# CX9898/BSMR-SDDMM

Measured on AMD Instinct MI355X. Metric: SDDMM GFLOP/s, higher is better.
Workload: dtype f16

## Files before the change

### bsmr-sddmm_amd/csrc/bsmr_capi.hip

```cpp

#include "bsmr_hip.h"

#include <hip/hip_runtime.h>
#include <hipcub/hipcub.hpp>

#include <algorithm>
#include <chrono>
#include <cmath>
#include <cstdio>
#include <cstdlib>
#include <cstring>
#include <map>
#include <memory>
#include <mutex>
#include <new>
#include <set>
#include <string>
#include <vector>

#include "cluster_kernels.hpp"
#include "pack_device.hpp"
#include "promote_device.hpp"
#include "plan_pack.hpp"
#include "plan_promote.hpp"
// ... 35 lines not shown
    uint32_t* groupRows = nullptr;
    uint32_t* blockCols = nullptr;
    uint32_t* blockInfo = nullptr;
    uint32_t* entries = nullptr;
    bsmr::TileItem* items = nullptr;
    uint32_t* itemRowBase = nullptr;
    uint32_t numItems = 0, entryCap = 0, blocksPerItem = 0;
    uint64_t numBlocks = 0, numTiles = 0, unionColumns = 0, bytes = 0;
};

struct SweepFormatDev {
    uint32_t W = 0, PW = 0, stripBlocks = 0;
    uint32_t* panelRows = nullptr;
    bsmr::SweepItem* items = nullptr;
    uint32_t* starts = nullptr;
    uint32_t* rowStart = nullptr;
    uint32_t* words = nullptr;
    uint32_t numItems = 0, numGroups = 0, numStrips = 0, maxStepEntries = 0, maxItemWords = 0;
    uint64_t bytes = 0;
    bool usable = false;
};

struct GemmFormatDev {
    uint32_t PM = 0, NB = 0;
    uint32_t* panelRows = nullptr;
    uint32_t* colOf = nullptr;
    bsmr::GemmItem* items = nullptr;
    uint32_t* rowStart = nullptr;
    uint32_t* lists = nullptr;
    uint32_t* words = nullptr;
    uint32_t numItems = 0, numGroups = 0, numStrips = 0;
    uint64_t numTiles = 0, bytes = 0;
    bool fullGrid = false, usable = false;
};

struct bsmr_plan {
    int device = 0;
    uint32_t M = 0, N = 0, nnz = 0, numPanels = 0;

    DenseFormat fmt[2];
    uint64_t numDenseEntries = 0;

    uint32_t* panelRows = nullptr;
    uint32_t* entryCol = nullptr;
    uint32_t* entryDst = nullptr;
    uint8_t* entryRow = nullptr;
    SparseItem* sparseItems = nullptr;
    uint64_t numSparseEntries = 0;
    uint32_t numSparseItems = 0;

    uint64_t indexBytes = 0;

    uint16_t* A16 = nullptr;
    uint16_t* B16 = nullptr;
    uint32_t reservedK = 0;

    int sparseLpe = 0;
    bool sparseLowp = true;
    bool convertInKernel = false;
    uint32_t* entryRowId = nullptr;
    bool sparseFree = false;
    uint64_t foldedEntries = 0;
    uint64_t promotedEntries = 0;
    uint64_t evictedEntries = 0;
    bool groupedDeferred = false;
    bsmr::PackOptions groupedOpt;
    float buildMs[5] = {0, 0, 0, 0, 0};
    bool packedOnDevice = false;
    bool promotedOnDevice = false;
    bool convertPass = false;
    bool convertBOnly = false;
    uint64_t bOnlyWork = 0;
    int denseBatch = 0;
    bool useStream = true;

    bsmr::HostDense hostDense;
    mutable bsmr::TileCensus census[5];
    mutable bool censusDone[5] = {false, false, false, false, false};
    TileFormatDev tiles[5];
    bool useTiles = false;
    bool sharedB = false;
    bool tunable = false;
    std::vector<SweepFormatDev> sweeps;
    bool useSweep = false;
    int sweepNow = -1;
    int sweepPanelsNow = 0, sweepBlocksNow = 0, sweepWavesNow = 0, sweepPerCuNow = 0;
    std::vector<GemmFormatDev> gemms;
    bool useGemm = false;
    int gemmNow = -1;
    int gemmPanelsNow = 0, gemmBlocksNow = 0;
    struct Tuned {
        int engine = BSMR_ENGINE_STREAM, group = 0, blocksPerItem = 0;
        int format = -1;
        int bOnly = -1;
        int overlap = -1;
        int cvt = -1;
        int waves = 0;
    };
    std::map<uint64_t, Tuned> tuned;
    int tileGroupNow = 0, tileBlocksNow = 0;
    int formatNow = -1, bOnlyNow = -1, overlapNow = -1, cvtNow = -1;
    bsmr_plan_options opt{};

    bool overlap = false;
    hipStream_t sideStream = nullptr;
    hipEvent_t forkEvent = nullptr, joinEvent = nullptr;

    struct Retained {
        bsmr_rphm_desc desc{};
        std::vector<uint32_t> reorderedRows, denseCols, blockOffsets, blockValues, sparseOffsets, sparseValues, sparseRows, sparseCols;
    };
    std::unique_ptr<Retained> retained;
    bsmr_plan* delegate = nullptr;
    uint64_t delegateKey = 0;
    int variantChosen = 0;
};

namespace {

constexpr uint64_t kGroupedGatherBytes = 400ull << 20;

thread_local std::string g_lastHipError;
inline bsmr_plan* served(bsmr_plan* p) { return p && p->delegate ? p->delegate : p; }
// ... 1071 lines not shown
    if (src32) {
        switch (K) {
        case 32: return launchSweepP<1, MODE, true>(w, p->device, perCu, p->N, A, B, P, s);
        case 64: return launchSweepP<2, MODE, true>(w, p->device, perCu, p->N, A, B, P, s);
        case 128: return launchSweepP<4, MODE, true>(w, p->device, perCu, p->N, A, B, P, s);
        default: return BSMR_ERR_INVALID_ARG;
        }
    }
    switch (K) {
    case 32: return launchSweepP<1, MODE, false>(w, p->device, perCu, p->N, A, B, P, s);
    case 64: return launchSweepP<2, MODE, false>(w, p->device, perCu, p->N, A, B, P, s);
    case 128: return launchSweepP<4, MODE, false>(w, p->device, perCu, p->N, A, B, P, s);
    case 256: return launchSweepP<8, MODE, false>(w, p->device, perCu, p->N, A, B, P, s);
    case 512: return launchSweepP<16, MODE, false>(w, p->device, perCu, p->N, A, B, P, s);
    default: return BSMR_ERR_INVALID_ARG;
    }
}

inline bool gemmServesK(uint32_t K) { return K == 64 || K == 128 || K == 256 || K == 512; }
inline bool gemmFp32ServesK(uint32_t K) { return K == 64 || K == 128; }
inline bool gemmFits(const bsmr_plan* p, uint32_t K, uint32_t elemBytes = 2) {
    return (uint64_t)p->M * K * elemBytes < (1ull << 32) && (uint64_t)p->N * K * elemBytes < (1ull << 32) &&
           (uint64_t)p->nnz * 4u <= 0xFFFFFFFCull;
}
inline bool gemmWanted(const bsmr_plan* p, uint32_t K) {
    return p->useGemm && gemmServesK(K) && gemmFits(p, K) && p->hostDense.entries() != 0;
}
inline bool gemmEngine(const bsmr_plan* p) { return p->gemmNow >= 0; }
inline bool gemmFp32(const bsmr_plan* p, uint32_t K) {
    if (!gemmFp32ServesK(K) || !gemmFits(p, K, 4)) return false;
    if (p->cvtNow >= 0) return p->cvtNow == 1;
    return p->opt.gemm_fp32 > 0 || (p->opt.gemm_fp32 < 0 && p->numSparseItems == 0);
}
constexpr uint32_t kGemmShapes[][2] = {{16, 16}, {16, 20}, {16, 12}, {8, 16}, {8, 20}};
inline double gemmModelUs(const bsmr_plan* p, uint32_t K, uint32_t PM, uint32_t NB) {
    const uint64_t G = (p->numPanels + PM - 1) / PM, S = ((p->N + 15u) / 16u + NB - 1) / NB;
    const double perCu = PM * NB <= 160 ? 2.0 : 1.0;
    const double rounds = std::ceil((double)(G * S) / (256.0 * perCu));
    const double slice = 1.4 * (PM * NB / 256.0) * (PM * NB < 256 ? 1.15 : 1.0) * perCu;
    return 2.0 + rounds * (4.0 + slice * (K / 64.0));
}
inline bool gemmShapeBuilt(uint32_t PM, uint32_t NB, bool fp32 = false) {
    for (const auto& sh : kGemmShapes)
        if (sh[0] == PM && sh[1] == NB) return !(fp32 && NB == 12);
    return false;
}
void gemmShape(const bsmr_plan* p, uint32_t K, uint32_t& PM, uint32_t& NB, int rank = 0) {
    const int forcedPM = p->gemmPanelsNow > 0 ? p->gemmPanelsNow : p->opt.gemm_panels;
    const int forcedNB = p->gemmBlocksNow > 0 ? p->gemmBlocksNow : p->opt.gemm_blocks;
    if (forcedPM > 0 && forcedNB > 0) {
        PM = (uint32_t)forcedPM;
        NB = (uint32_t)forcedNB;
        return;
    }
    std::vector<std::pair<double, uint32_t>> order;
    const bool fp32 = gemmFp32(p, K);
    for (uint32_t i = 0; i < sizeof(kGemmShapes) / sizeof(kGemmShapes[0]); ++i)
        if (gemmShapeBuilt(kGemmShapes[i][0], kGemmShapes[i][1], fp32))
            order.push_back({gemmModelUs(p, K, kGemmShapes[i][0], kGemmShapes[i][1]), i});
    std::stable_sort(order.begin(), order.end());
    const uint32_t pick = order[std::min<size_t>((size_t)rank, order.size() - 1)].second;
    PM = kGemmShapes[pick][0];
    NB = kGemmShapes[pick][1];
}

int ensureGemm(bsmr_plan* p, uint32_t K) {
    uint32_t PM, NB;
    gemmShape(p, K, PM, NB);
    p->gemmNow = -1;
    if (!gemmShapeBuilt(PM, NB, gemmFp32(p, K))) return BSMR_OK;
    for (size_t i = 0; i < p->gemms.size(); ++i)
        if (p->gemms[i].PM == PM && p->gemms[i].NB == NB) {
            if (p->gemms[i].usable) p->gemmNow = (int)i;
            return BSMR_OK;
        }
    try {
        GemmFormatDev w;
        w.PM = PM;
        w.NB = NB;
        bsmr::GemmFormatHost host;
        int st = bsmr::packGemm(p->hostDense, PM, NB, host, p->opt.gemm_balance_columns != 0);
        if (st == BSMR_ERR_BAD_PLAN || st == BSMR_ERR_INVALID_ARG) {
            p->gemms.push_back(w);
            return BSMR_OK;
        }
        if (st != BSMR_OK) return st;
        uint64_t bytes = 0;
        w.numItems = (uint32_t)host.items.size();
        w.numGroups = host.numGroups;
        w.numStrips = host.numStrips;
        w.numTiles = host.numTiles;
        w.fullGrid = host.fullGrid;
        st = upload(w.panelRows, host.panelRows, bytes);
        if (st == BSMR_OK) st = upload(w.colOf, host.colOf, bytes);
        if (st == BSMR_OK) st = upload(w.items, host.items, bytes);
        if (st == BSMR_OK) st = upload(w.rowStart, host.rowStart, bytes);
        if (st == BSMR_OK) st = upload(w.lists, host.lists, bytes);
        if (st == BSMR_OK) st = upload(w.words, host.words, bytes);
        if (st != BSMR_OK) {
            void* wp[] = {w.panelRows, w.colOf, w.items, w.rowStart, w.lists, w.words};
            for (void* q : wp)
                if (q) (void)hipFree(q);
            return st;
        }
        w.bytes = bytes;
        w.usable = w.numItems != 0;
        p->indexBytes += bytes;
        p->gemms.push_back(w);
        if (w.usable) p->gemmNow = (int)p->gemms.size() - 1;
        return BSMR_OK;
    } catch (const std::bad_alloc&) {
        return BSMR_ERR_OOM;
    }
}

template <int KT, int PM, int NB, int MODE, bool SRC32>
int launchGemmT(const GemmFormatDev& w, const bsmr_plan* p, const void* A, const void* B, float* P, const Queue& s) {
    const uint64_t K = (SRC32 ? 32u : 64u) * KT, esz = SRC32 ? 4 : 2;
    const uint32_t aBytes = (uint32_t)((uint64_t)p->M * K * esz), bBytes = (uint32_t)((uint64_t)p->N * K * esz);
    const dim3 grid(w.numItems, s.batch.count), block(bsmr::kGemmWaves * bsmr::kWave);
    if constexpr (SRC32) {
        auto kernel = bsmr::denseGemmCvt<KT, PM, NB, MODE>;
        const size_t lds = bsmr::gemmCvtLdsBytes(PM, NB);
        if (int st = raiseDynamicLds(reinterpret_cast<const void*>(kernel), lds, p->device)) return st;
        hipLaunchKernelGGL(kernel, grid, block, lds, s, static_cast<const float*>(A), static_cast<const float*>(B), aBytes, bBytes, w.panelRows,
                           w.colOf, w.items, w.rowStart, w.lists, w.words, P, p->N, w.numGroups, w.numStrips, w.fullGrid ? 1u : 0u, s.batch);
    } else {
        auto kernel = bsmr::denseGemm<KT, PM, NB, MODE, false>;
        const size_t lds = bsmr::gemmLdsBytes(PM, NB);
        if (int st = raiseDynamicLds(reinterpret_cast<const void*>(kernel), lds, p->device)) return st;
        hipLaunchKernelGGL(kernel, grid, block, lds, s, A, B, aBytes, bBytes, w.panelRows, w.colOf, w.items, w.rowStart, w.lists, w.words, P, p->N,
                           w.numGroups, w.numStrips, w.fullGrid ? 1u : 0u, s.batch);
    }
    BSMR_HIP(hipGetLastError());
    return BSMR_OK;
}
template <int KT, int MODE, bool SRC32>
int launchGemmS(const GemmFormatDev& w, const bsmr_plan* p, const void* A, const void* B, float* P, const Queue& s) {
    switch (w.PM * 100 + w.NB) {
    case 1616: return launchGemmT<KT, 16, 16, MODE, SRC32>(w, p, A, B, P, s);
    case 1620: return launchGemmT<KT, 16, 20, MODE, SRC32>(w, p, A, B, P, s);
    case 816: return launchGemmT<KT, 8, 16, MODE, SRC32>(w, p, A, B, P, s);
    case 820: return launchGemmT<KT, 8, 20, MODE, SRC32>(w, p, A, B, P, s);
    case 1612:
        if constexpr (!SRC32) return launchGemmT<KT, 16, 12, MODE, false>(w, p, A, B, P, s);
        return BSMR_ERR_INVALID_ARG;
    default: return BSMR_ERR_INVALID_ARG;
    }
}
template <int MODE>
int launchGemm(const bsmr_plan* p, uint32_t K, const void* A, const void* B, float* P, const Queue& s, bool src32) {
    const GemmFormatDev& w = p->gemms[(size_t)p->gemmNow];
    if (w.numItems == 0) return BSMR_OK;
    if (src32) {
        switch (K) {
        case 64: return launchGemmS<2, MODE, true>(w, p, A, B, P, s);
        case 128: return launchGemmS<4, MODE, true>(w, p, A, B, P, s);
        default: return BSMR_ERR_INVALID_ARG;
        }
    }
    switch (K) {
    case 64: return launchGemmS<1, MODE, false>(w, p, A, B, P, s);
    case 128: return launchGemmS<2, MODE, false>(w, p, A, B, P, s);
    case 256: return launchGemmS<4, MODE, false>(w, p, A, B, P, s);
    case 512: return launchGemmS<8, MODE, false>(w, p, A, B, P, s);
    default: return BSMR_ERR_INVALID_ARG;
    }
}

inline bool streamCvtServes(const DenseFormat& f, uint32_t K) {
    return (K == 32 || K == 64 || K == 128) && f.H == 1 && f.maxItemBlocks <= 8 && (f.tiles8 || f.tilesM) && !f.stageInLds;
// ... 221 lines not shown
        return BSMR_ERR_INVALID_ARG;
    return BSMR_OK;
}

bool aligned16(const void* p) { return ((uintptr_t)p & 15u) == 0; }
bool aligned4(const void* p) { return ((uintptr_t)p & 3u) == 0; }

int checkDeviceCall(const bsmr_plan* p, uint32_t K, const void* A, const void* B, const void* P, int mode) {
    if (int st = checkCall(p, K, A, B, P, mode)) return st;
    return aligned16(A) && aligned16(B) && aligned4(P) ? BSMR_OK : BSMR_ERR_INVALID_ARG;
}

inline bool convertsBOnly(const bsmr_plan* p, uint32_t K, uint32_t batches = 1) {
    if (!p->convertBOnly || (size_t)16 * (2u * K + bsmr::kSparseLdsPad16) > 64 * 1024) return false;
    if (p->bOnlyNow >= 0) return p->bOnlyNow == 1;
    const uint64_t work = (uint64_t)p->numSparseEntries * K * batches;
    return work >= p->bOnlyWork || (p->numSparseEntries >= 11ull * p->N && work * 10 >= p->bOnlyWork * 3);
}

inline bool needsWorkspace(const bsmr_plan* p, int mode, uint32_t K, uint32_t batches = 1) {
    return mode != BSMR_COMPUTE_F32 && (convertPassOf(p, K) || convertsBOnly(p, K, batches));
}

int prepareDense(bsmr_plan* p, uint32_t K, int mode) {
    p->sweepNow = -1;
    p->gemmNow = -1;
    if (p->tunable) {
        const auto it = mode == BSMR_COMPUTE_F32 ? p->tuned.end() : p->tuned.find(((uint64_t)K << 8) | (uint32_t)mode);
        const bsmr_plan::Tuned choice = it == p->tuned.end() ? bsmr_plan::Tuned{} : it->second;
        p->useSweep = choice.engine == BSMR_ENGINE_SWEEP;
        p->useGemm = choice.engine == BSMR_ENGINE_GEMM;
        p->gemmPanelsNow = p->useGemm ? choice.group : 0;
        p->gemmBlocksNow = p->useGemm ? choice.blocksPerItem : 0;
        p->useTiles = choice.engine == BSMR_ENGINE_TILES || choice.engine == BSMR_ENGINE_SHARED;
        p->sharedB = choice.engine == BSMR_ENGINE_SHARED;
        p->tileGroupNow = p->useTiles ? choice.group : 0;
        p->tileBlocksNow = p->useTiles ? choice.blocksPerItem : 0;
        p->sweepPanelsNow = p->useSweep ? choice.group : 0;
        p->sweepBlocksNow = p->useSweep ? choice.blocksPerItem : 0;
        p->sweepWavesNow = p->useSweep ? choice.waves : 0;
        p->formatNow = choice.format;
        p->bOnlyNow = choice.bOnly;
        p->overlapNow = choice.overlap;
        p->cvtNow = choice.cvt;
    }
    if (mode == BSMR_COMPUTE_F32) return BSMR_OK;
    if (gemmWanted(p, K)) {
        if (int st = ensureGemm(p, K)) return st;
        if (gemmEngine(p)) return BSMR_OK;
    }
    if (sweepWanted(p, K)) {
        if (int st = ensureSweep(p, K)) return st;
        if (sweepEngine(p)) return BSMR_OK;
    }
    if (!tilesEngine(p, K)) return BSMR_OK;
    return ensureTiles(p, chooseTileGroup(p, K));
}

int reserve(bsmr_plan* p, uint32_t K) {
    if (p->reservedK >= K && p->A16 && p->B16) return BSMR_OK;
    if (p->A16) (void)hipFree(p->A16);
    if (p->B16) (void)hipFree(p->B16);
    p->A16 = p->B16 = nullptr;
    p->reservedK = 0;
    const size_t a = std::max<size_t>((size_t)p->M * K * 2, 16), b = std::max<size_t>((size_t)p->N * K * 2, 16);
    if (!hipOk(hipMalloc(reinterpret_cast<void**>(&p->A16), a), "hipMalloc(A16)")) return BSMR_ERR_OOM;
// ... 1124 lines not shown
        }
        if (st == BSMR_OK && r.lowp_call_us >= 0.f && r.sweep_fp32_call_us >= 0.f && r.sweep_fp32_call_us < r.lowp_call_us * kTuneMargin) {
            best = bestF;
            r.chosen_sweep_fp32 = 1;
        }
    }
    if (st == BSMR_OK && lowp && gemmFp32ServesK(K) && gemmFits(plan, K, 4) && plan->fmt[0].numItems && !plan->convertInKernel && sweepApplies(plan)) {
        float callUs = r.lowp_call_us;
        if (r.chosen_sweep_fp32 && r.sweep_fp32_call_us >= 0.f) callUs = r.sweep_fp32_call_us;
        if (callUs < 0.f) st = timeChoice(best, 7, callUs);
        bsmr_plan::Tuned f = best, bestF = best;
        f.engine = BSMR_ENGINE_GEMM;
        f.format = -1;
        f.cvt = 1;
        f.waves = 0;
        uint32_t seenPM = 0, seenNB = 0;
        for (int rank = 0; rank < 2 && st == BSMR_OK; ++rank) {
            uint32_t PM, NB;
            plan->gemmPanelsNow = plan->gemmBlocksNow = 0;
            plan->cvtNow = 1;
            gemmShape(plan, K, PM, NB, rank);
            if (PM == seenPM && NB == seenNB) continue;
            seenPM = PM;
            seenNB = NB;
            f.group = (int)PM;
            f.blocksPerItem = (int)NB;
            float us = -1.f;
            st = timeChoice(f, 7, us);
            if (st == BSMR_OK && us >= 0.f && (r.gemm_fp32_call_us < 0.f || us < r.gemm_fp32_call_us)) {
                r.gemm_fp32_call_us = us;
                bestF = f;
            }
        }
        if (st == BSMR_OK && callUs >= 0.f && r.gemm_fp32_call_us >= 0.f && r.gemm_fp32_call_us < callUs * kTuneMargin) {
            best = bestF;
            r.chosen_sweep_fp32 = 0;
            r.chosen_gemm_fp32 = 1;
        }
        if (r.lowp_call_us < 0.f) r.lowp_call_us = callUs;
    }
    if (st != BSMR_OK) {
        plan->tuned.erase(key);
        return st;
    }
    plan->tuned[key] = best;
    r.chosen_cvt_in_kernel = best.cvt;
    r.chosen_engine = best.engine;
    r.chosen_group = best.engine == BSMR_ENGINE_STREAM ? (best.format == 1 ? (int)plan->fmt[1].H : 1) : best.group;
    r.chosen_blocks_per_item = best.blocksPerItem;
    r.chosen_b_only = best.bOnly;
    r.chosen_overlap = best.overlap;
    if ((st = prepareDense(plan, K, mode)) != BSMR_OK) return st;
    if (best.engine == BSMR_ENGINE_SWEEP && sweepEngine(plan)) r.chosen_blocks_per_item = (int)plan->sweeps[(size_t)plan->sweepNow].stripBlocks;
    if (needsWorkspace(plan, mode, K) && (st = reserve(plan, K)) != BSMR_OK) return st;
    st = runPieces(plan, K, A, B, P, mode, s, 7);
    if (st == BSMR_OK && report) *report = r;
    return st;
}

int timeWholeCalls(bsmr_plan* plan, uint32_t K, const float* A, const float* B, float* P, int mode, hipStream_t s, float* us) {
    hipEvent_t e0 = nullptr, e1 = nullptr;
    BSMR_HIP(hipEventCreate(&e0));
    if (!hipOk(hipEventCreate(&e1), "hipEventCreate")) {
        (void)hipEventDestroy(e0);
        return BSMR_ERR_HIP;
    }
    int st = BSMR_OK;
    float best = 1e30f;
    for (int rep = 0; rep < 3 && st == BSMR_OK; ++rep) {
        const int iters = 30;
// ... 28 lines not shown
                   bsmr_tune_report* report) {
    return bsmr_plan_tune_sized(plan, K, A, B, P, mode, stream, report, sizeof(bsmr_tune_report));
}

int bsmr_plan_tune_sized(bsmr_plan* plan, uint32_t K, const float* A, const float* B, float* P, int mode, void* stream,
                         bsmr_tune_report* report, size_t report_size) {
    bsmr_tune_report r{};
    const int st = tunePlan(plan, K, A, B, P, mode, stream, &r);
    if (st == BSMR_OK && report) memcpy(report, &r, std::min(report_size, sizeof(r)));
    return st;
}

int bsmr_plan_get_tuned(const bsmr_plan* plan, uint32_t K, int mode, bsmr_tuned_choice* out) {
    plan = served(plan);
    if (!plan || !out || !plan->tunable) return BSMR_ERR_INVALID_ARG;
    const auto it = plan->tuned.find(((uint64_t)K << 8) | (uint32_t)mode);
    if (it == plan->tuned.end()) return BSMR_ERR_INVALID_ARG;
    *out = choiceOf(it->second);
    return BSMR_OK;
}

int bsmr_plan_set_tuned(bsmr_plan* plan, uint32_t K, int mode, const bsmr_tuned_choice* choice) {
    plan = served(plan);
    if (!plan || !choice || !plan->tunable || choice->struct_size < sizeof(bsmr_tuned_choice)) return BSMR_ERR_INVALID_ARG;
    if (K == 0 || (K & 31u)) return BSMR_ERR_UNSUPPORTED_K;
    if (mode != BSMR_COMPUTE_F16 && mode != BSMR_COMPUTE_BF16) return BSMR_ERR_INVALID_ARG;
    bsmr_plan::Tuned t;
    t.engine = choice->engine; t.group = choice->group; t.blocksPerItem = choice->blocks_per_item; t.format = choice->format;
    t.bOnly = choice->b_only; t.overlap = choice->overlap; t.cvt = choice->cvt_in_kernel; t.waves = choice->waves;
    const bool engineOk = t.engine == BSMR_ENGINE_STREAM || t.engine == BSMR_ENGINE_TILES || t.engine == BSMR_ENGINE_SHARED ||
                          t.engine == BSMR_ENGINE_SWEEP || t.engine == BSMR_ENGINE_GEMM;
    if (!engineOk || t.group < 0 || t.blocksPerItem < 0 || t.format < -1 || t.format > 1 || t.bOnly < -1 || t.bOnly > 1 ||
        t.overlap < -1 || t.overlap > 1 || t.cvt < -1 || t.cvt > 1 || t.waves < 0)
        return BSMR_ERR_INVALID_ARG;
    if (t.format == 1 && !plan->fmt[1].H && plan->groupedDeferred) {
        BSMR_HIP(hipSetDevice(plan->device));
        const int gs = ensureGrouped(plan);
        if (gs != BSMR_OK) return gs;
    }
    if (t.format == 1 && !plan->fmt[1].H) return BSMR_ERR_BAD_PLAN;
    if ((t.engine == BSMR_ENGINE_TILES || t.engine == BSMR_ENGINE_SHARED) && (!tilesServeK(K) || plan->hostDense.entries() == 0)) return BSMR_ERR_BAD_PLAN;
    if (t.engine == BSMR_ENGINE_SWEEP && (!sweepServesK(K) || plan->hostDense.entries() == 0)) return BSMR_ERR_BAD_PLAN;
    if (t.engine == BSMR_ENGINE_GEMM && (!gemmServesK(K) || plan->hostDense.entries() == 0)) return BSMR_ERR_BAD_PLAN;
    if (t.cvt == 1 && !(t.engine == BSMR_ENGINE_SWEEP ? K <= 128 : t.engine == BSMR_ENGINE_GEMM ? (gemmFp32ServesK(K) && gemmFits(plan, K, 4)) : streamCvtServes(plan->fmt[0], K)))
        return BSMR_ERR_BAD_PLAN;
    BSMR_HIP(hipSetDevice(plan->device));
    const uint64_t key = ((uint64_t)K << 8) | (uint32_t)mode;
    const auto before = plan->tuned.find(key);
    const bool had = before != plan->tuned.end();
    const bsmr_plan::Tuned old = had ? before->second : bsmr_plan::Tuned{};
    plan->tuned[key] = t;
    int st = prepareDense(plan, K, mode);
    if (st == BSMR_OK && t.engine == BSMR_ENGINE_SWEEP && !sweepEngine(plan)) st = BSMR_ERR_BAD_PLAN;
    if (st == BSMR_OK && t.engine == BSMR_ENGINE_GEMM && !gemmEngine(plan)) st = BSMR_ERR_BAD_PLAN;
    if (st == BSMR_OK && needsWorkspace(plan, mode, K)) st = reserve(plan, K);
    if (st != BSMR_OK) {
        if (had) plan->tuned[key] = old;
        else plan->tuned.erase(key);
        (void)prepareDense(plan, K, mode);
    }
    return st;
}

namespace {
int tunePlan(bsmr_plan* plan, uint32_t K, const float* A, const float* B, float* P, int mode, void* stream,
             bsmr_tune_report* report) {
// ... 438 lines not shown
```

### bsmr-sddmm_amd/csrc/gemm_format.hpp

```cpp
#pragma once

#include <algorithm>
#include <cstdint>
#include <vector>

#include "bsmr_hip.h"
#include "tile_format.hpp"

namespace bsmr {

constexpr uint32_t kGemmWavesM = 2, kGemmWavesN = 4, kGemmWaves = kGemmWavesM * kGemmWavesN;
__host__ __device__ constexpr uint32_t gemmSlabSlot(uint32_t tp, uint32_t r, uint32_t c) { return tp * 256u + (r & 3u) * 64u + (r >> 2) * 16u + c; }
constexpr uint32_t kGemmPassTiles = 16;
constexpr uint32_t kGemmNoEntry = 0xFFFFFFFFu;
constexpr uint32_t kGemmMaxOffset = 8191u;
constexpr uint32_t kGemmSlabStrips = 8;
constexpr uint32_t kGemmWordSlack = 1024;

struct GemmItem {
    uint32_t group;
    uint32_t firstBlock;
    uint32_t listBase;
    uint32_t pad;
};

__host__ __device__ inline void gemmItemPlace(uint32_t i, uint32_t G, uint32_t S, uint32_t& group, uint32_t& strip) {
    const uint32_t slabs = (S + kGemmSlabStrips - 1u) / kGemmSlabStrips;
    uint32_t slab = i / (kGemmSlabStrips * G);
    if (slab >= slabs) slab = slabs - 1u;
    const uint32_t width = slab + 1u < slabs ? kGemmSlabStrips : S - kGemmSlabStrips * (slabs - 1u);
    const uint32_t rem = i - slab * kGemmSlabStrips * G;
    group = rem / width;
    strip = slab * kGemmSlabStrips + rem % width;
}

struct GemmFormatHost {
    uint32_t PM = 0, NB = 0, numGroups = 0, numStrips = 0, passes = 0;
    bool fullGrid = false;
    std::vector<uint32_t> panelRows;
    std::vector<uint32_t> colOf;
    std::vector<GemmItem> items;
    std::vector<uint32_t> rowStart;
    std::vector<uint32_t> lists;
    std::vector<uint32_t> words;
    uint64_t numTiles = 0;
    uint32_t maxListWords = 0;
    size_t bytes() const {
        return 4 * (panelRows.size() + colOf.size() + rowStart.size() + lists.size() + words.size()) + sizeof(GemmItem) * items.size();
    }
};

inline bool gemmShapeOk(uint32_t PM, uint32_t NB) {
    return (PM == 8 || PM == 16) && (NB == 8 || NB == 12 || NB == 16 || NB == 20);
}

inline int packGemm(const HostDense& hd, uint32_t PM, uint32_t NB, GemmFormatHost& out, bool balanceColumns = true) {
    if (!gemmShapeOk(PM, NB)) return BSMR_ERR_INVALID_ARG;
    const uint32_t P = hd.numPanels, TM = PM * 16;
    const uint32_t G = (P + PM - 1) / PM, NCB = (hd.N + 15) / 16, S = (NCB + NB - 1) / NB;
    const uint32_t m = PM / kGemmWavesM, n = NB / kGemmWavesN, Q = (m * n + kGemmPassTiles - 1) / kGemmPassTiles, L = kGemmWaves * Q;
    out = GemmFormatHost();
    out.PM = PM; out.NB = NB; out.numGroups = G; out.numStrips = S; out.passes = Q;
    if (P == 0 || NCB == 0 || hd.entries() == 0) return BSMR_OK;
    if ((uint64_t)G * S > 0x3FFFFFFFull || hd.entries() > 0xFFFFFFF0ull) return BSMR_ERR_INVALID_ARG;
    if ((uint64_t)hd.nnz * 4u > 0xFFFFFFFCull) return BSMR_ERR_INVALID_ARG;
    out.panelRows.assign((size_t)G * TM, hd.panelRows.empty() ? 0u : hd.panelRows[0]);
    std::vector<uint32_t> rowPos((size_t)P * 16);
    if (balanceColumns) {
        std::vector<uint32_t> weight((size_t)P * 16, 0), order((size_t)P * 16);
        for (uint32_t p = 0; p < P; ++p)
            for (uint64_t e = hd.offsets[p]; e < hd.offsets[p + 1]; ++e) ++weight[(size_t)p * 16 + hd.row[e]];
        for (uint32_t i = 0; i < P * 16; ++i) order[i] = i;
        std::stable_sort(order.begin(), order.end(), [&](uint32_t a, uint32_t b) { return weight[a] > weight[b]; });
        const uint32_t bins = 2 * G, half = TM / 2;
        for (uint32_t rank = 0; rank < P * 16; ++rank) {
            const uint32_t round = rank / bins, pos = rank % bins, bin = (round & 1u) ? bins - 1u - pos : pos;
            rowPos[order[rank]] = (bin / 2) * TM + (bin % 2) * half + round;
        }
    } else {
        for (uint32_t i = 0; i < P * 16; ++i) rowPos[i] = i;
    }
    for (uint32_t i = 0; i < P * 16; ++i) out.panelRows[rowPos[i]] = hd.panelRows[i];
    const uint32_t TN = NB * 16;
    std::vector<uint32_t> slotOf(hd.N);
    out.colOf.assign((size_t)S * TN, 0u);
    if (balanceColumns) {
        std::vector<uint32_t> degree(hd.N, 0), hot;
        for (uint64_t e = 0; e < hd.entries(); ++e) ++degree[hd.col[e]];
        uint64_t fullest = 0;
        for (uint32_t st = 0; st < S; ++st) {
            uint64_t sum = 0;
            for (uint32_t c = st * TN; c < std::min<uint64_t>(hd.N, (uint64_t)(st + 1) * TN); ++c) sum += degree[c];
            fullest = std::max(fullest, sum);
        }
        const bool lopsided = fullest * S > 2ull * hd.entries();
// ... 15 lines not shown
    } else {
        for (uint32_t c = 0; c < hd.N; ++c) slotOf[c] = c;
    }
    for (uint32_t c = 0; c < hd.N; ++c) out.colOf[slotOf[c]] = c;
    std::vector<uint32_t> itemOf((size_t)G * S, 0xFFFFFFFFu);
    std::vector<uint8_t> used((size_t)G * S, 0);
    for (uint32_t p = 0; p < P; ++p)
        for (uint64_t e = hd.offsets[p]; e < hd.offsets[p + 1]; ++e)
            used[(size_t)(rowPos[(size_t)p * 16 + hd.row[e]] / TM) * S + slotOf[hd.col[e]] / TN] = 1;
    for (uint32_t i = 0; i < G * S; ++i) {
        uint32_t g, st;
        gemmItemPlace(i, G, S, g, st);
        if (!used[(size_t)g * S + st]) continue;
        itemOf[(size_t)g * S + st] = (uint32_t)out.items.size();
        GemmItem it;
        it.group = g;
        it.firstBlock = st * NB;
        it.listBase = (uint32_t)(out.items.size() * (L + 1));
        it.pad = 0;
        out.items.push_back(it);
    }
    out.fullGrid = out.items.size() == (size_t)G * S;
    const size_t I = out.items.size();
    out.numTiles = (uint64_t)I * PM * NB;
    if (I * (size_t)(L + 1) > 0xFFFFFFFFull || I * (size_t)TM > 0xFFFFFFFFull) return BSMR_ERR_INVALID_ARG;
    out.lists.assign(I * (L + 1), 0);
    out.rowStart.assign(I * TM, 0xFFFFFFFFu);
    auto locate = [&](uint32_t p, uint64_t e, size_t& item, uint32_t& list, uint32_t& slot, uint32_t& rowInWave, uint32_t& rowInTile) {
        const uint32_t place = rowPos[(size_t)p * 16 + hd.row[e]];
        const uint32_t g = place / TM, pj = (place % TM) / 16u;
        const uint32_t slotCol = slotOf[hd.col[e]];
        const uint32_t cb = slotCol >> 4, s = cb / NB, bj = cb % NB;
        const uint32_t wm = pj / m, tm = pj % m, wn = bj / n, tn = bj % n;
        const uint32_t t = tm * n + tn, q = t / kGemmPassTiles, tp = t % kGemmPassTiles;
        const uint32_t r = place & 15u, c = slotCol & 15u;
        item = itemOf[(size_t)g * S + s];
        list = (wm * kGemmWavesN + wn) * Q + q;
        slot = gemmSlabSlot(tp, r, c);
        rowInWave = tm * 16 + r;
        rowInTile = pj * 16 + r;
    };
    for (uint32_t p = 0; p < P; ++p)
        for (uint64_t e = hd.offsets[p]; e < hd.offsets[p + 1]; ++e) {
            size_t item; uint32_t list, slot, rw, rt;
            locate(p, e, item, list, slot, rw, rt);
            ++out.lists[item * (L + 1) + list + 1];
            uint32_t& rs = out.rowStart[item * TM + rt];
            rs = std::min(rs, hd.idx[e]);
        }
    for (uint32_t& v : out.rowStart)
        if (v == 0xFFFFFFFFu) v = 0;
    uint64_t at = 0;
    for (size_t item = 0; item < I; ++item) {
        uint32_t* ls = &out.lists[item * (L + 1)];
        uint64_t run = at;
        for (uint32_t l = 0; l <= L; ++l) {
            const uint32_t cnt = ls[l];
            out.maxListWords = std::max(out.maxListWords, (cnt + 3u) & ~3u);
            run += (cnt + 3u) & ~3u;
            if (run > 0xFFFFFFF0ull) return BSMR_ERR_INVALID_ARG;
            ls[l] = (uint32_t)run;
        }
        at = run;
    }
    if (at > 0xFFFFFFF0ull) return BSMR_ERR_INVALID_ARG;
    out.words.assign((size_t)at + kGemmWordSlack, kGemmNoEntry);
    std::vector<uint32_t> fill(out.lists.size());
// ... 28 lines not shown
```

### bsmr-sddmm_amd/csrc/gemm_kernels.hpp

```cpp
#pragma once

#include <hip/hip_runtime.h>
#include <stdint.h>

#include "gemm_format.hpp"
#include "sddmm_kernels.hpp"

namespace bsmr {

constexpr uint32_t kGemmBK = 64;
constexpr uint32_t kGemmRowBytes = kGemmBK * 2u;
__host__ __device__ constexpr uint32_t gemmSwz16(uint32_t row) { return (row >> 1) & 7u; }
__host__ __device__ constexpr uint32_t gemmSwz32(uint32_t row) { return ((row >> 1) & 1u) | (((row >> 3) & 1u) * 6u); }
constexpr uint32_t gemmStageBytes(int PM, int NB) { return (uint32_t)(PM + NB) * 16u * kGemmRowBytes; }
constexpr uint32_t kGemmSlabBytes = kGemmPassTiles * 1024u;
constexpr uint32_t gemmRingBytes(int PM, int NB) {
    return 2u * gemmStageBytes(PM, NB) > kGemmWaves * kGemmSlabBytes ? 2u * gemmStageBytes(PM, NB) : kGemmWaves * kGemmSlabBytes;
}
constexpr size_t gemmLdsBytes(int PM, int NB) { return gemmRingBytes(PM, NB) + (size_t)PM * 16u * 4u; }

#if defined(BSMR_GEMM_LAB)
#define GEMM_LAB_ARG , uint32_t labSkip, unsigned long long* labStamps
#define GEMM_LAB_SKIP(bit) (labSkip & (1u << (bit)))
#define GEMM_LAB_STAMPS unsigned long long labStamp[8] = {0, 0, 0, 0, 0, 0, 0, 0}
// ... 452 lines not shown
        }
        const uint32_t first = myList[q], last = myList[q + 1u];
        uint32_t w[kGemmWordChunk];
#pragma unroll
        for (uint32_t u = 0; u < kGemmWordChunk; ++u) w[u] = wAhead[q & 1u][u];
        if (kDeepWords) {
            if (q + 2u < Q) loadWords(myList[q + 2u], wAhead[q & 1u]);
        } else if (q + 1u < Q) {
            loadWords(last, wAhead[(q + 1u) & 1u]);
        }
        for (uint32_t e = first; e < last; e += kGemmWordChunk * kWave) {
            if (e != first) loadWords(e, w);
#pragma unroll
            for (uint32_t u = 0; u < kGemmWordChunk; ++u) {
#if defined(BSMR_GEMM_BRANCHY_STORES)
                if (e + u * kWave + lane < last && w[u] != kGemmNoEntry) {
                    const float val = slab[w[u] & 4095u];
                    const uint32_t dst = rowTable[(w[u] >> 12) & 127u] + (w[u] >> 19);
                    if (!GEMM_LAB_SKIP(5)) P[dst] = val;
                }
#else
                const bool live = e + u * kWave + lane < last && w[u] != kGemmNoEntry;
                const float val = slab[w[u] & 4095u];
                const uint32_t dst = rowTable[(w[u] >> 12) & (TM / 2u - 1u)] + (w[u] >> 19);
                if (!GEMM_LAB_SKIP(5)) gemmStoreEntry(P, live, dst, val);
#endif
            }
        }
        GEMM_LAB_STAMP(5u + q);
    }
    GEMM_LAB_STAMPS_OUT;
}

}
```

Measured before the change: 15460.

## Add paired-occupancy fp32-convert GEMM kernel with smaller LDS and pass tiles

Adds a specialised 8x16 fp32-source GEMM SDDMM kernel that streams fp32 rows in half-K pieces through a smaller LDS ring and converts them to f16/bf16 in place. It uses 8-tile output passes so that two workgroups fit per CU. The packer gains a passTiles parameter, and the autotuner gets a new candidate (waves==2) for this variant. The aim is higher occupancy and better latency hiding for the fp32-input path. The cost is more conversion turns and extra barriers per K step.

```diff
diff --git a/bsmr-sddmm_amd/csrc/bsmr_capi.hip b/bsmr-sddmm_amd/csrc/bsmr_capi.hip
--- a/bsmr-sddmm_amd/csrc/bsmr_capi.hip
+++ b/bsmr-sddmm_amd/csrc/bsmr_capi.hip
@@ -91,6 +91,7 @@
     uint32_t numItems = 0, numGroups = 0, numStrips = 0;
     uint64_t numTiles = 0, bytes = 0;
     bool fullGrid = false, usable = false;
+    uint32_t passTiles = bsmr::kGemmPassTiles;
 };
 
 struct bsmr_plan {
@@ -148,6 +149,7 @@
     bool useGemm = false;
     int gemmNow = -1;
     int gemmPanelsNow = 0, gemmBlocksNow = 0;
+    bool gemmPairNow = false;
     struct Tuned {
         int engine = BSMR_ENGINE_STREAM, group = 0, blocksPerItem = 0;
         int format = -1;
@@ -1285,6 +1287,10 @@
     if (p->cvtNow >= 0) return p->cvtNow == 1;
     return p->opt.gemm_fp32 > 0 || (p->opt.gemm_fp32 < 0 && p->numSparseItems == 0);
 }
+inline bool gemmPaired(const bsmr_plan* p, uint32_t K, uint32_t PM, uint32_t NB) {
+    if (PM != bsmr::kGemmPairPM || NB != bsmr::kGemmPairNB || !gemmFp32(p, K)) return false;
+    return p->cvtNow >= 0 ? p->gemmPairNow : p->opt.gemm_fp32 == 2;
+}
 constexpr uint32_t kGemmShapes[][2] = {{16, 16}, {16, 20}, {16, 12}, {8, 16}, {8, 20}};
 inline double gemmModelUs(const bsmr_plan* p, uint32_t K, uint32_t PM, uint32_t NB) {
     const uint64_t G = (p->numPanels + PM - 1) / PM, S = ((p->N + 15u) / 16u + NB - 1) / NB;
@@ -1322,8 +1328,9 @@
     gemmShape(p, K, PM, NB);
     p->gemmNow = -1;
     if (!gemmShapeBuilt(PM, NB, gemmFp32(p, K))) return BSMR_OK;
+    const uint32_t passTiles = gemmPaired(p, K, PM, NB) ? bsmr::kGemmPairPassTiles : bsmr::kGemmPassTiles;
     for (size_t i = 0; i < p->gemms.size(); ++i)
-        if (p->gemms[i].PM == PM && p->gemms[i].NB == NB) {
+        if (p->gemms[i].PM == PM && p->gemms[i].NB == NB && p->gemms[i].passTiles == passTiles) {
             if (p->gemms[i].usable) p->gemmNow = (int)i;
             return BSMR_OK;
         }
@@ -1331,8 +1338,9 @@
         GemmFormatDev w;
         w.PM = PM;
         w.NB = NB;
+        w.passTiles = passTiles;
         bsmr::GemmFormatHost host;
-        int st = bsmr::packGemm(p->hostDense, PM, NB, host, p->opt.gemm_balance_columns != 0);
+        int st = bsmr::packGemm(p->hostDense, PM, NB, host, p->opt.gemm_balance_columns != 0, passTiles);
         if (st == BSMR_ERR_BAD_PLAN || st == BSMR_ERR_INVALID_ARG) {
             p->gemms.push_back(w);
             return BSMR_OK;
@@ -1388,8 +1396,28 @@
     BSMR_HIP(hipGetLastError());
     return BSMR_OK;
 }
+template <int KT, int MODE>
+int launchGemmPair(const GemmFormatDev& w, const bsmr_plan* p, const void* A, const void* B, float* P, const Queue& s) {
+    const uint64_t K = 32u * KT;
+    const uint32_t aBytes = (uint32_t)((uint64_t)p->M * K * 4u), bBytes = (uint32_t)((uint64_t)p->N * K * 4u);
+    const dim3 grid(w.numItems, s.batch.count), block(bsmr::kGemmWaves * bsmr::kWave);
+    auto kernel = bsmr::denseGemmCvtPair<KT, MODE>;
+    const size_t lds = bsmr::kGemmPairLdsBytes;
+    if (int st = raiseDynamicLds(reinterpret_cast<const void*>(kernel), lds, p->device)) return st;
+    hipLaunchKernelGGL(kernel, grid, block, lds, s, static_cast<const float*>(A), static_cast<const float*>(B), aBytes, bBytes, w.panelRows,
+                       w.colOf, w.items, w.rowStart, w.lists, w.words, P, p->N, w.numGroups, w.numStrips, w.fullGrid ? 1u : 0u, s.batch);
+    BSMR_HIP(hipGetLastError());
+    return BSMR_OK;
+}
 template <int KT, int MODE, bool SRC32>
 int launchGemmS(const GemmFormatDev& w, const bsmr_plan* p, const void* A, const void* B, float* P, const Queue& s) {
+    if (w.passTiles != bsmr::kGemmPassTiles) {
+        if constexpr (SRC32) {
+            if (w.PM == bsmr::kGemmPairPM && w.NB == bsmr::kGemmPairNB && w.passTiles == bsmr::kGemmPairPassTiles)
+                return launchGemmPair<KT, MODE>(w, p, A, B, P, s);
+        }
+        return BSMR_ERR_INVALID_ARG;
+    }
     switch (w.PM * 100 + w.NB) {
     case 1616: return launchGemmT<KT, 16, 16, MODE, SRC32>(w, p, A, B, P, s);
     case 1620: return launchGemmT<KT, 16, 20, MODE, SRC32>(w, p, A, B, P, s);
@@ -1677,6 +1705,7 @@
         p->useGemm = choice.engine == BSMR_ENGINE_GEMM;
         p->gemmPanelsNow = p->useGemm ? choice.group : 0;
         p->gemmBlocksNow = p->useGemm ? choice.blocksPerItem : 0;
+        p->gemmPairNow = p->useGemm && choice.waves == 2;
         p->useTiles = choice.engine == BSMR_ENGINE_TILES || choice.engine == BSMR_ENGINE_SHARED;
         p->sharedB = choice.engine == BSMR_ENGINE_SHARED;
         p->tileGroupNow = p->useTiles ? choice.group : 0;
@@ -2867,10 +2896,21 @@
                 bestF = f;
             }
         }
+        if (st == BSMR_OK) {
+            f.group = (int)bsmr::kGemmPairPM;
+            f.blocksPerItem = (int)bsmr::kGemmPairNB;
+            f.waves = 2;
+            float us = -1.f;
+            st = timeChoice(f, 7, us);
+            if (st == BSMR_OK && us >= 0.f && (r.gemm_fp32_call_us < 0.f || us < r.gemm_fp32_call_us * kTuneMargin)) {
+                r.gemm_fp32_call_us = us;
+                bestF = f;
+            }
+        }
         if (st == BSMR_OK && callUs >= 0.f && r.gemm_fp32_call_us >= 0.f && r.gemm_fp32_call_us < callUs * kTuneMargin) {
             best = bestF;
             r.chosen_sweep_fp32 = 0;
-            r.chosen_gemm_fp32 = 1;
+            r.chosen_gemm_fp32 = bestF.waves == 2 ? 2 : 1;
         }
         if (r.lowp_call_us < 0.f) r.lowp_call_us = callUs;
     }
@@ -2965,6 +3005,8 @@
                           t.engine == BSMR_ENGINE_SWEEP || t.engine == BSMR_ENGINE_GEMM;
     if (!engineOk || t.group < 0 || t.blocksPerItem < 0 || t.format < -1 || t.format > 1 || t.bOnly < -1 || t.bOnly > 1 ||
         t.overlap < -1 || t.overlap > 1 || t.cvt < -1 || t.cvt > 1 || t.waves < 0)
+        return BSMR_ERR_INVALID_ARG;
+    if (t.engine == BSMR_ENGINE_GEMM && t.waves == 2 && (t.group != (int)bsmr::kGemmPairPM || t.blocksPerItem != (int)bsmr::kGemmPairNB || t.cvt != 1))
         return BSMR_ERR_INVALID_ARG;
     if (t.format == 1 && !plan->fmt[1].H && plan->groupedDeferred) {
         BSMR_HIP(hipSetDevice(plan->device));
diff --git a/bsmr-sddmm_amd/csrc/gemm_format.hpp b/bsmr-sddmm_amd/csrc/gemm_format.hpp
--- a/bsmr-sddmm_amd/csrc/gemm_format.hpp
+++ b/bsmr-sddmm_amd/csrc/gemm_format.hpp
@@ -12,6 +12,7 @@
 constexpr uint32_t kGemmWavesM = 2, kGemmWavesN = 4, kGemmWaves = kGemmWavesM * kGemmWavesN;
 __host__ __device__ constexpr uint32_t gemmSlabSlot(uint32_t tp, uint32_t r, uint32_t c) { return tp * 256u + (r & 3u) * 64u + (r >> 2) * 16u + c; }
 constexpr uint32_t kGemmPassTiles = 16;
+constexpr uint32_t kGemmPairPassTiles = 8, kGemmPairPM = 8, kGemmPairNB = 16;
 constexpr uint32_t kGemmNoEntry = 0xFFFFFFFFu;
 constexpr uint32_t kGemmMaxOffset = 8191u;
 constexpr uint32_t kGemmSlabStrips = 8;
@@ -35,7 +36,7 @@
 }
 
 struct GemmFormatHost {
-    uint32_t PM = 0, NB = 0, numGroups = 0, numStrips = 0, passes = 0;
+    uint32_t PM = 0, NB = 0, numGroups = 0, numStrips = 0, passes = 0, passTiles = kGemmPassTiles;
     bool fullGrid = false;
     std::vector<uint32_t> panelRows;
     std::vector<uint32_t> colOf;
@@ -54,13 +55,14 @@
     return (PM == 8 || PM == 16) && (NB == 8 || NB == 12 || NB == 16 || NB == 20);
 }
 
-inline int packGemm(const HostDense& hd, uint32_t PM, uint32_t NB, GemmFormatHost& out, bool balanceColumns = true) {
-    if (!gemmShapeOk(PM, NB)) return BSMR_ERR_INVALID_ARG;
+inline int packGemm(const HostDense& hd, uint32_t PM, uint32_t NB, GemmFormatHost& out, bool balanceColumns = true,
+                    uint32_t passTiles = kGemmPassTiles) {
+    if (!gemmShapeOk(PM, NB) || (passTiles != kGemmPassTiles && passTiles != kGemmPairPassTiles)) return BSMR_ERR_INVALID_ARG;
     const uint32_t P = hd.numPanels, TM = PM * 16;
     const uint32_t G = (P + PM - 1) / PM, NCB = (hd.N + 15) / 16, S = (NCB + NB - 1) / NB;
-    const uint32_t m = PM / kGemmWavesM, n = NB / kGemmWavesN, Q = (m * n + kGemmPassTiles - 1) / kGemmPassTiles, L = kGemmWaves * Q;
+    const uint32_t m = PM / kGemmWavesM, n = NB / kGemmWavesN, Q = (m * n + passTiles - 1) / passTiles, L = kGemmWaves * Q;
     out = GemmFormatHost();
-    out.PM = PM; out.NB = NB; out.numGroups = G; out.numStrips = S; out.passes = Q;
+    out.PM = PM; out.NB = NB; out.numGroups = G; out.numStrips = S; out.passes = Q; out.passTiles = passTiles;
     if (P == 0 || NCB == 0 || hd.entries() == 0) return BSMR_OK;
     if ((uint64_t)G * S > 0x3FFFFFFFull || hd.entries() > 0xFFFFFFF0ull) return BSMR_ERR_INVALID_ARG;
     if ((uint64_t)hd.nnz * 4u > 0xFFFFFFFCull) return BSMR_ERR_INVALID_ARG;
@@ -142,7 +144,7 @@
         const uint32_t slotCol = slotOf[hd.col[e]];
         const uint32_t cb = slotCol >> 4, s = cb / NB, bj = cb % NB;
         const uint32_t wm = pj / m, tm = pj % m, wn = bj / n, tn = bj % n;
-        const uint32_t t = tm * n + tn, q = t / kGemmPassTiles, tp = t % kGemmPassTiles;
+        const uint32_t t = tm * n + tn, q = t / passTiles, tp = t % passTiles;
         const uint32_t r = place & 15u, c = slotCol & 15u;
         item = itemOf[(size_t)g * S + s];
         list = (wm * kGemmWavesN + wn) * Q + q;
diff --git a/bsmr-sddmm_amd/csrc/gemm_kernels.hpp b/bsmr-sddmm_amd/csrc/gemm_kernels.hpp
--- a/bsmr-sddmm_amd/csrc/gemm_kernels.hpp
+++ b/bsmr-sddmm_amd/csrc/gemm_kernels.hpp
@@ -508,4 +508,209 @@
     GEMM_LAB_STAMPS_OUT;
 }
 
-}
+constexpr uint32_t kGemmPairFRowBytes = 64u;
+constexpr uint32_t kGemmPairRows = (kGemmPairPM + kGemmPairNB) * 16u;
+constexpr uint32_t kGemmPairSlabBytes = kGemmPairPassTiles * 1024u;
+constexpr uint32_t kGemmPairRingBytes = kGemmPairRows * (kGemmPairFRowBytes + 2u * kGemmHalfRowBytes);
+constexpr size_t kGemmPairLdsBytes = kGemmPairRingBytes + kGemmPairPM * 16u * 4u;
+static_assert(kGemmWaves * kGemmPairSlabBytes <= 0x10000u && kGemmWaves * kGemmPairSlabBytes <= kGemmPairRingBytes,
+              "the slabs lie inside the dead ring and below 64 KiB (ds_write_addtid: M0 holds 16 bits)");
+static_assert(2u * ((kGemmPairLdsBytes + 1279u) / 1280u * 1280u) <= 160u * 1024u, "two workgroups' LDS fits a CU");
+
+__device__ __forceinline__ uint32_t gemmRowOfLane16(const uint32_t* __restrict__ rows16, uint32_t sub) {
+    uint32_t id = rows16[0];
+#pragma unroll
+    for (uint32_t k = 1; k < 16; ++k) id = sub == k ? rows16[k] : id;
+    return id;
+}
+
+#if defined(BSMR_GEMM_LAB)
+#define GEMM_LAB_PLACE labStamp[7] = ((unsigned long long)__builtin_amdgcn_s_getreg(63508) << 32) | __builtin_amdgcn_s_getreg(63492)
+#else
+#define GEMM_LAB_PLACE
+#endif
+
+template <int KT, int MODE>
+__global__ void __launch_bounds__(kGemmWaves * kWave, 4)
+denseGemmCvtPair(const float* __restrict__ Aop, const float* __restrict__ Bop, uint32_t aBytes, uint32_t bBytes,
+                 const uint32_t* __restrict__ panelRows, const uint32_t* __restrict__ colOf, const GemmItem* __restrict__ items,
+                 const uint32_t* __restrict__ rowStart,
+                 const uint32_t* __restrict__ lists, const uint32_t* __restrict__ words, float* __restrict__ P, uint32_t N,
+                 uint32_t gridG, uint32_t gridS, uint32_t fullGrid, Batch batch GEMM_LAB_ARG) {
+    constexpr uint32_t PM = kGemmPairPM, NB = kGemmPairNB, PT = kGemmPairPassTiles;
+    constexpr uint32_t K = 32u * KT, TM = PM * 16u, TN = NB * 16u, ROWS = kGemmPairRows;
+    constexpr uint32_t m = PM / kGemmWavesM, n = NB / kGemmWavesN, Q = (m * n + PT - 1u) / PT, L = kGemmWaves * Q;
+    constexpr uint32_t CHUNKS = ROWS / 16u / kGemmWaves, ACHUNKS = TM / 16u;
+    static_assert(CHUNKS * 16u * kGemmWaves == ROWS, "F is filled in whole 1-KiB pieces per wave");
+    constexpr uint32_t fBytes = ROWS * kGemmPairFRowBytes, hBytes = ROWS * kGemmHalfRowBytes, bAtH = TM * kGemmHalfRowBytes;
+    constexpr uint32_t hAt = fBytes, rowTableAt = kGemmPairRingBytes;
+    constexpr uint32_t kGemmWordChunk = 4u;
+
+    extern __shared__ __attribute__((aligned(16))) uint8_t lds[];
+    const uint32_t itemId = xcdContiguous(blockIdx.x, gridDim.x);
+    uint32_t group, firstBlock, listBase;
+    if (fullGrid) {
+        gemmItemPlace(itemId, gridG, gridS, group, firstBlock);
+        firstBlock *= NB;
+        listBase = itemId * (L + 1u);
+    } else {
+        const GemmItem item = items[itemId];
+        group = item.group;
+        firstBlock = item.firstBlock;
+        listBase = item.listBase;
+    }
+    const uint32_t wave = __builtin_amdgcn_readfirstlane(threadIdx.x >> 6), lane = threadIdx.x & 63u;
+    const uint32_t wm = wave / kGemmWavesN, wn = wave % kGemmWavesN;
+    const uint32_t r = lane & 15u, g = lane >> 4;
+    GEMM_LAB_STAMPS;
+    GEMM_LAB_STAMP(0);
+    GEMM_LAB_PLACE;
+    const uint8_t* Ab = reinterpret_cast<const uint8_t*>(Aop) + (size_t)blockIdx.y * batch.strideA * 4u;
+    const uint8_t* Bb = reinterpret_cast<const uint8_t*>(Bop) + (size_t)blockIdx.y * batch.strideB * 4u;
+    P += (size_t)blockIdx.y * batch.strideP;
+
+    uint32_t voff[CHUNKS];
+#pragma unroll
+    for (uint32_t j = 0; j < CHUNKS; ++j) {
+        const uint32_t c = wave * CHUNKS + j;
+        const uint32_t* ids = c < ACHUNKS ? panelRows + (size_t)group * TM + 16u * c : colOf + (size_t)firstBlock * 16u + 16u * (c - ACHUNKS);
+        voff[j] = gemmRowOfLane16(ids, lane >> 2) * (K * 4u) + ((lane & 3u) << 4);
+    }
+    auto refill = [&](uint32_t rf) {
+        if (GEMM_LAB_SKIP(2)) return;
+#pragma unroll
+        for (uint32_t j = 0; j < CHUNKS; ++j) {
+            const uint32_t c = wave * CHUNKS + j;
+            const auto rsrc = __builtin_amdgcn_make_buffer_rsrc(const_cast<uint8_t*>(c < ACHUNKS ? Ab : Bb), 0, c < ACHUNKS ? aBytes : bBytes, 0x00020000);
+            __builtin_amdgcn_raw_ptr_buffer_load_lds(rsrc, (__attribute__((address_space(3))) void*)(lds + c * 1024u), 16, voff[j], rf * kGemmPairFRowBytes, 0, 0);
+        }
+    };
+    refill(0u);
+    GEMM_LAB_STAMP(1);
+    if (threadIdx.x < TM) reinterpret_cast<uint32_t*>(lds + rowTableAt)[threadIdx.x] = rowStart[(size_t)itemId * TM + threadIdx.x];
+    uint32_t myList[Q + 1];
+#pragma unroll
+    for (uint32_t q = 0; q <= Q; ++q) myList[q] = lists[listBase + wave * Q + q];
+
+    const uint32_t fOf = wave * CHUNKS * 1024u + lane * 16u;
+    const uint32_t hOf = hAt + (wave * CHUNKS * 16u + (lane >> 2)) * kGemmHalfRowBytes + ((((lane & 3u) >> 1) ^ gemmSwzH(lane >> 2)) << 4) + ((lane & 1u) << 3);
+    auto roundChunks = [&](uint32_t to, uint32_t half) {
+        if (GEMM_LAB_SKIP(1)) return;
+        f32x4 v[CHUNKS];
+#pragma unroll
+        for (uint32_t j = 0; j < CHUNKS; ++j) v[j] = *reinterpret_cast<const f32x4*>(lds + fOf + j * 1024u);
+#pragma unroll
+        for (uint32_t j = 0; j < CHUNKS; ++j) {
+            uint8_t* dst = lds + (hOf ^ (half << 5)) + j * 1024u + to * hBytes;
+            typedef uint32_t u32x2 __attribute__((ext_vector_type(2)));
+            u32x2 h;
+            if constexpr (MODE == 0) {
+                typedef _Float16 f16x4 __attribute__((ext_vector_type(4)));
+                f16x4 o;
+                o[0] = (_Float16)v[j][0]; o[1] = (_Float16)v[j][1]; o[2] = (_Float16)v[j][2]; o[3] = (_Float16)v[j][3];
+                h = __builtin_bit_cast(u32x2, o);
+            } else {
+                typedef __bf16 bf16x4 __attribute__((ext_vector_type(4)));
+                bf16x4 o;
+                o[0] = (__bf16)v[j][0]; o[1] = (__bf16)v[j][1]; o[2] = (__bf16)v[j][2]; o[3] = (__bf16)v[j][3];
+                h = __builtin_bit_cast(u32x2, o);
+            }
+            *reinterpret_cast<u32x2*>(dst) = h;
+        }
+    };
+    auto turn = [&](uint32_t rf) {
+        asm volatile("s_waitcnt vmcnt(0)" ::: "memory");
+        roundChunks((rf >> 1) & 1u, rf & 1u);
+        asm volatile("s_waitcnt lgkmcnt(0)" ::: "memory");
+        if (rf + 1u < 2u * (uint32_t)KT) refill(rf + 1u);
+    };
+
+    const uint32_t fragOff = r * kGemmHalfRowBytes + ((g ^ gemmSwzH(r)) << 4);
+    const uint32_t aRead = wm * (TM / 2u) * kGemmHalfRowBytes + fragOff;
+    const uint32_t bRead = bAtH + wn * (TN / 4u) * kGemmHalfRowBytes + fragOff;
+
+    f32x4 acc[m][n];
+#pragma unroll
+    for (uint32_t i = 0; i < m; ++i)
+#pragma unroll
+        for (uint32_t j = 0; j < n; ++j) acc[i][j] = f32x4{0.f, 0.f, 0.f, 0.f};
+    auto loadWords = [&](uint32_t e0, uint32_t (&w)[kGemmWordChunk]) {
+#pragma unroll
+        for (uint32_t u = 0; u < kGemmWordChunk; ++u) w[u] = GEMM_LAB_SKIP(4) ? kGemmNoEntry : words[e0 + u * kWave + lane];
+    };
+    uint32_t wAhead[Q][kGemmWordChunk];
+
+    asm volatile("s_waitcnt vmcnt(0)" ::: "memory");
+    GEMM_LAB_STAMP(2);
+    roundChunks(0u, 0u);
+    asm volatile("s_waitcnt lgkmcnt(0)" ::: "memory");
+    refill(1u);
+    turn(1u);
+    __builtin_amdgcn_s_barrier();
+    GEMM_LAB_STAMP(3);
+#pragma unroll
+    for (uint32_t q = 0; q < Q; ++q) loadWords(myList[q], wAhead[q]);
+
+#pragma unroll
+    for (uint32_t t = 0; t < (uint32_t)KT; ++t) {
+        const uint8_t* base = lds + hAt + (t & 1u) * hBytes;
+        u32x4 bf[n];
+#pragma unroll
+        for (uint32_t j = 0; j < n; ++j)
+            bf[j] = GEMM_LAB_SKIP(6) ? u32x4{lane, t, j, 0u} : *reinterpret_cast<const u32x4*>(base + bRead + j * 16u * kGemmHalfRowBytes);
+#pragma unroll
+        for (uint32_t i = 0; i < m; ++i) {
+            const u32x4 af = GEMM_LAB_SKIP(6) ? u32x4{lane, t, i, 2u} : *reinterpret_cast<const u32x4*>(base + aRead + i * 16u * kGemmHalfRowBytes);
+            if (!GEMM_LAB_SKIP(0)) {
+#pragma unroll
+                for (uint32_t j = 0; j < n; ++j) acc[i][j] = mfma16<MODE>(af, bf[j], acc[i][j]);
+            } else {
+                gemmKeep(af);
+#pragma unroll
+                for (uint32_t j = 0; j < n; ++j) gemmKeep(bf[j]);
+            }
+            if (t + 1u < (uint32_t)KT) {
+                if (i == m / 2u - 1u) turn(2u * t + 2u);
+                if (i == m - 1u) turn(2u * t + 3u);
+            }
+        }
+        asm volatile("s_waitcnt lgkmcnt(0)" ::: "memory");
+        __builtin_amdgcn_s_barrier();
+    }
+
+    __builtin_amdgcn_sched_barrier(0);
+    asm volatile("s_nop 15\n\ts_nop 15\n\ts_nop 15" ::: "memory");
+    __builtin_amdgcn_sched_barrier(0);
+    GEMM_LAB_STAMP(4);
+    float* slab = reinterpret_cast<float*>(lds) + wave * (PT * 256u);
+    const uint32_t slabAddr = __builtin_amdgcn_readfirstlane(gemmLdsAddress(slab));
+    const uint32_t* rowTable = reinterpret_cast<const uint32_t*>(lds + rowTableAt) + wm * (TM / 2u);
+#pragma unroll
+    for (uint32_t q = 0; q < Q; ++q) {
+        if (!GEMM_LAB_SKIP(3)) {
+#pragma unroll
+            for (uint32_t tp = 0; tp < PT; ++tp) {
+                const uint32_t tIdx = q * PT + tp;
+                if (tIdx < m * n) gemmDumpTile(acc[tIdx / n][tIdx % n], slabAddr + tp * 1024u, false);
+            }
+        }
+        const uint32_t first = myList[q], last = myList[q + 1u];
+        uint32_t w[kGemmWordChunk];
+#pragma unroll
+        for (uint32_t u = 0; u < kGemmWordChunk; ++u) w[u] = wAhead[q][u];
+        for (uint32_t e = first; e < last; e += kGemmWordChunk * kWave) {
+            if (e != first) loadWords(e, w);
+#pragma unroll
+            for (uint32_t u = 0; u < kGemmWordChunk; ++u) {
+                const bool live = e + u * kWave + lane < last && w[u] != kGemmNoEntry;
+                const float val = slab[w[u] & (PT * 256u - 1u)];
+                const uint32_t dst = rowTable[(w[u] >> 12) & (TM / 2u - 1u)] + (w[u] >> 19);
+                if (!GEMM_LAB_SKIP(5)) gemmStoreEntry(P, live, dst, val);
+            }
+        }
+        GEMM_LAB_STAMP(5u + q);
+    }
+    GEMM_LAB_STAMPS_OUT;
+}
+
+}
```

Result: slower. 13940 (-9.8%).
